# eukaryo/smith-waterman-simd

Measured on AMD Instinct MI355X. Metric: alignments/sec (and GCUPS) on 1M fixed-length pairs, 1/2/4/8 MI355X, higher is better.
Workload: dtype u16

## Files before the change

smith-waterman-simd_amd/csrc/swmi_api.cpp:

```cpp
#include "swmi_host.h"
#include "pk_form.h"

#include <cstdarg>
#include <cstdio>
#include <cstdlib>
#include <cstring>
#include <ctime>
#include <new>

namespace swmi {
namespace host {

namespace {
thread_local char t_error[512] = "";
thread_local int t_status = SWMI_OK;
thread_local int t_gpu = 0;
std::vector<std::shared_ptr<Context>> g_ctxs;
std::mutex g_init_mu;
Knobs g_knobs;
bool g_knobs_read = false;
std::atomic<uint64_t> g_schedule{0};
std::atomic<uint64_t> g_sg_mapping{0};
}

std::atomic<uint64_t> &sg_mapping_word() { return g_sg_mapping; }

int fail(int code, const char *fmt, ...)
{
    va_list ap;
    va_start(ap, fmt);
    vsnprintf(t_error, sizeof t_error, fmt, ap);
    va_end(ap);
    t_status = code;
    return code;
}

int last_status() { return t_status; }

std::mutex &init_mutex() { return g_init_mu; }
int num_contexts() { return (int)g_ctxs.size(); }
Context *context_at(int index) { return index >= 0 && index < (int)g_ctxs.size() ? g_ctxs[index].get() : nullptr; }
std::shared_ptr<Context> context_ref(int index) { return index >= 0 && index < (int)g_ctxs.size() ? g_ctxs[index] : nullptr; }

int check_alive(const Context &ctx)
{
    if (!ctx.dead.load(std::memory_order_acquire)) return SWMI_OK;
    return fail(SWMI_ERR_NOT_INITIALIZED, "swmi_shutdown() ran after this handle was created: only its *_destroy call is valid now");
}

const Knobs &knobs() { return g_knobs; }

void read_knobs()
{
    Knobs k;
    auto num = [](const char *name, long long lo, long long hi, long long dflt) {
        const char *v = getenv(name);
        if (!v || !*v) return dflt;
        const long long x = atoll(v);
        return x < lo || x > hi ? dflt : x;
    };
    k.host_granule = (size_t)num("SWMI_HOST_GRANULE", 1024, (long long)kChunkPairs, 0);
    k.host_serial = num("SWMI_HOST_SERIAL", 0, 1, 0) != 0;
    k.host_taper_pct = (unsigned)num("SWMI_HOST_TAPER", 1, 99, 0);
    k.host_min_granule = (size_t)num("SWMI_HOST_MIN_GRANULE", 1024, (long long)kChunkPairs, 0);
    if (const char *sched = getenv("SWMI_HOST_SCHEDULE")) {
        int c = 0;
        for (const char *q = sched; *q && c < 16;) {
            char *end = nullptr;
            const long long v = strtoll(q, &end, 10);
            if (end == q) break;
            if (v >= 1024 && v <= (long long)kChunkPairs) k.host_schedule[c++] = (size_t)v;
            q = *end == ',' ? end + 1 : end;
        }
    }
    k.host_trace = num("SWMI_HOST_TRACE", 0, 1, 0) != 0;
    k.host_threads = (int)num("SWMI_HOST_THREADS", 1, kHostThreads, 0);
    k.host_slots = (int)num("SWMI_HOST_SLOTS", 2, kSlots / kHostThreads, 0);
    k.score_group = (size_t)num("SWMI_TEST_SCORE_GROUP", 4096, (long long)kScoreGroup, (long long)kScoreGroup);
    k.extra_lds = (unsigned)num("SWMI_EXTRA_LDS", 0, 160 * 1024, 0);
    k.lanes = (int)num("SWMI_LANES", 0, 64, 0);
    k.banded_no_i16 = getenv("SWMI_BANDED_NO_I16") != nullptr;
    k.banded_no_pk = getenv("SWMI_BANDED_NO_PK") != nullptr;
    k.pk_no_product = getenv("SWMI_PK_NO_PRODUCT") != nullptr;
    k.sg_sweep = (int)num("SWMI_SG_SWEEP", 1, 44, -1);
    k.sg_exact = (int)num("SWMI_SG_EXACT", 0, 1, -1);
    const char *gb = getenv("SWMI_GATHER_BACKEND");
    k.gather_p2p = gb && strcmp(gb, "p2p") == 0;
    k.gather_piece = (size_t)num("SWMI_TEST_GATHER_PIECE", 1, 1ll << 40, 0);
    if (const char *lib = getenv("SWMI_RCCL_LIB")) snprintf(k.rccl_lib, sizeof k.rccl_lib, "%s", lib);
    g_knobs = k;
    g_knobs_read = true;
}

Context *current()
{
    if (g_ctxs.empty()) {
        fail(SWMI_ERR_NOT_INITIALIZED, "swmi_init() has not been called (or failed)");
        return nullptr;
    }
    Context *ctx = context_at(t_gpu);
    if (!ctx) {
        fail(SWMI_ERR_INVALID_ARGUMENT, "this thread selected GPU index %d but only %d are bound", t_gpu, (int)g_ctxs.size());
        return nullptr;
    }
    const hipError_t e = hipSetDevice(ctx->device);
    if (e != hipSuccess) {
        fail(SWMI_ERR_HIP, "hipSetDevice(%d) failed: %s", ctx->device, hipGetErrorString(e));
        return nullptr;
    }
    return ctx;
}

int check_params(const int8_t *sm, int gap)
{
    if (!sm) return fail(SWMI_ERR_INVALID_ARGUMENT, "score_matrix is NULL");
    if (gap < 0) return fail(SWMI_ERR_DOMAIN, "gap_penalty %d < 0 is outside the supported domain [0,127]", gap);
    return SWMI_OK;
}

SmRows pack_rows(const int8_t *sm, int add)
{
    SmRows rows;
    for (int a = 0; a < 4; ++a) {
        uint32_t r = 0;
        for (int b = 0; b < 4; ++b) r |= uint32_t(uint8_t(int8_t(sm[4 * a + b] + add))) << (8 * b);
        rows.r[a] = r;
    }
    return rows;
}

namespace {
int auto_lanes(size_t n)
{
    return n <= 2048 ? 64 : n <= 5120 ? 32 : n <= 24576 ? 16 : n <= 98304 ? 8 : 4;
}
int resolve_lanes(uint64_t schedule, size_t n)
{
    const int lanes = int(schedule & 0xffffffffu);
    const unsigned flags = unsigned(schedule >> 32);
    return lanes ? lanes : (flags & swmi::kUseLut) ? 4 : auto_lanes(n);
}
}

LaunchConfig make_config(const Context &ctx, const int8_t *sm, int gap, SmRows *rows, size_t n)
{
    const uint64_t schedule = g_schedule.load(std::memory_order_relaxed);
    const unsigned flags = unsigned(schedule >> 32);
    LaunchConfig cfg;
    cfg.lanes_per_alignment = resolve_lanes(schedule, n);
    cfg.use_i16 = (flags & swmi::kUseI16) != 0;
    cfg.use_lut = (flags & swmi::kUseLut) != 0;
    cfg.extra_lds_bytes = ctx.extra_lds;
    cfg.pk_bias = 0;
    cfg.pk_variant = 0;
    bool fold = !(flags & swmi::kNoGapFold);
    for (int k = 0; k < 16 && fold; ++k) {
        const int v = int(sm[k]) + gap;
        if (v < -128 || v > 127) fold = false;
    }
    cfg.fold_gap = fold;
// ... 29 lines not shown
        }
        for (int a = 0; a < 4; ++a) {
            uint32_t r = 0;
            for (int b = 0; b < 4; ++b) r |= uint32_t(int(sm[4 * a + b]) + add) << (8 * b);
            rows->r[a] = r;
        }
        return cfg;
    }
    *rows = pack_rows(sm, fold ? gap : 0);
    return cfg;
}

namespace {
int ensure_slot(Slot &s, size_t bytes, size_t scores)
{
    if (s.capacity < bytes) {
        if (s.d_seq1) { (void)hipFree(s.d_seq1); s.d_seq1 = nullptr; }
        if (s.d_seq2) { (void)hipFree(s.d_seq2); s.d_seq2 = nullptr; }
        s.capacity = 0;
        SWMI_HIP_TRY(hipMalloc(&s.d_seq1, bytes));
        SWMI_HIP_TRY(hipMalloc(&s.d_seq2, bytes));
        s.capacity = bytes;
    }
    if (s.score_capacity < scores) {
        if (s.d_scores) { (void)hipFree(s.d_scores); s.d_scores = nullptr; }
        s.score_capacity = 0;
        SWMI_HIP_TRY(hipMalloc(reinterpret_cast<void **>(&s.d_scores), scores * sizeof(int32_t)));
        s.score_capacity = scores;
    }
    return SWMI_OK;
}

}

int launch_device(Context &ctx, const void *d1, const void *d2, size_t n, const int8_t *sm, int gap, void *d_out,
                  hipStream_t st, bool packed)
{
    SmRows rows;
    const LaunchConfig cfg = make_config(ctx, sm, gap, &rows, n);
    const size_t stride = packed ? SWMI_PACKED_LEN : kSeq;
    for (size_t off = 0; off < n; off += kMaxLaunchPairs) {
        const size_t m = n - off < kMaxLaunchPairs ? n - off : kMaxLaunchPairs;
        SWMI_HIP_TRY(swmi::launch_score(cfg, static_cast<const uint8_t *>(d1) + off * stride,
                                        static_cast<const uint8_t *>(d2) + off * stride,
                                        static_cast<int32_t *>(d_out) + off, m, rows, gap, packed, st));
    }
    return SWMI_OK;
}

size_t host_entry_bytes(int entry)
{
    return entry == kEntryPacked ? 2 * SWMI_PACKED_LEN : entry == kEntryOneVsMany ? kSeq : 2 * kSeq;
}

size_t next_granule(size_t remaining, size_t bytes_per_pair)
{
    const Knobs &kn = knobs();
    if (kn.host_granule) return remaining < kn.host_granule ? remaining : kn.host_granule;
    const size_t smallest = kn.host_min_granule ? kn.host_min_granule : kMinGranule;
    if (remaining <= smallest) return remaining;
    size_t f1024 = kn.host_taper_pct ? size_t(kn.host_taper_pct) * 1024 / 100 : 65536 / bytes_per_pair;
    if (f1024 > kMaxTaper1024) f1024 = kMaxTaper1024;
    size_t g = (remaining - remaining * f1024 / 1024) & ~size_t(4095);
    if (g > kChunkPairs) g = kChunkPairs;
    if (g < smallest) g = smallest;
    return g;
}

namespace {
int ensure_scores_all(Context &ctx, size_t pairs)
{
    if (ctx.scores_all_capacity >= pairs) return SWMI_OK;
    if (ctx.d_scores_all) { (void)hipFree(ctx.d_scores_all); ctx.d_scores_all = nullptr; }
    ctx.scores_all_capacity = 0;
    SWMI_HIP_TRY(hipMalloc(reinterpret_cast<void **>(&ctx.d_scores_all), pairs * sizeof(int32_t)));
    ctx.scores_all_capacity = pairs;
    return SWMI_OK;
}
}

namespace {
struct Granule { size_t off, m; };

struct TraceRow { size_t index, pairs; int thread; hipEvent_t ev[3]; double host_issue_ms[2]; };
std::mutex g_trace_mu;
std::vector<TraceRow> g_trace;
double host_now_ms()
{
    timespec ts;
    clock_gettime(CLOCK_MONOTONIC, &ts);
    return ts.tv_sec * 1e3 + ts.tv_nsec * 1e-6;
}

hipError_t issue_granules(Context &ctx, const std::vector<Granule> &list, size_t first, size_t step, Slot *const *slots, int n_slots,
                          const uint8_t *s1, const uint8_t *s2, size_t group, size_t in_stride, const int8_t *sm, int gap,
                          int32_t *out, bool packed, bool one_vs_many, bool serial, bool *slot_used, size_t early = 0,
                          bool *slot_early_used = nullptr, std::atomic<bool> *early_done = nullptr)
{
    hipError_t e = hipSuccess;
    size_t j = 0;
    for (size_t i = first; i < list.size() && e == hipSuccess; i += step, ++j) {
        const size_t off = list[i].off, m = list[i].m, at = group + off;
        const int which = int(j % size_t(n_slots));
        Slot &s = *slots[which];
        SmRows rows;
        const LaunchConfig cfg = make_config(ctx, sm, gap, &rows, m);
        TraceRow tr{i, m, int(first), {nullptr, nullptr, nullptr}, {0, 0}};
        const bool trace = knobs().host_trace;
        if (trace) {
            for (auto &ev : tr.ev) (void)hipEventCreate(&ev);
            tr.host_issue_ms[0] = host_now_ms();
            (void)hipEventRecord(tr.ev[0], s.stream);
        }
        e = hipMemcpyAsync(s.d_seq1, s1 + at * in_stride, m * in_stride, hipMemcpyHostToDevice, s.stream);
        if (e == hipSuccess && !one_vs_many)
            e = hipMemcpyAsync(s.d_seq2, s2 + at * in_stride, m * in_stride, hipMemcpyHostToDevice, s.stream);
        if (trace) (void)hipEventRecord(tr.ev[1], s.stream);
        if (e == hipSuccess)
            e = one_vs_many ? swmi::launch_score_one_vs_many(cfg, s.d_seq1, s.d_seq2, ctx.d_scores_all + off, m, rows, gap, s.stream)
                            : swmi::launch_score(cfg, s.d_seq1, s.d_seq2, ctx.d_scores_all + off, m, rows, gap, packed, s.stream);
        if (trace) {
            (void)hipEventRecord(tr.ev[2], s.stream);
            tr.host_issue_ms[1] = host_now_ms();
            std::lock_guard<std::mutex> l(g_trace_mu);
            g_trace.push_back(tr);
        }
        if (e == hipSuccess && serial)
            e = hipMemcpyAsync(out + at, ctx.d_scores_all + off, m * sizeof(int32_t), hipMemcpyDeviceToHost, s.stream);
        slot_used[which] = true;
        if (i < early && e == hipSuccess) {
            e = hipEventRecord(ctx.slot_early[&s - ctx.slots], s.stream);
            slot_early_used[which] = true;
        }
        if (early_done && i + step >= early) early_done->store(true, std::memory_order_release);
    }
    if (early_done) early_done->store(true, std::memory_order_release);
    return e;
}
}

void granule_list(size_t group_n, size_t bytes_per_pair, std::vector<size_t> *out)
{
    out->clear();
    const Knobs &kn = knobs();
    if (kn.host_schedule[0]) {
        size_t k = 0;
        for (size_t rem = group_n; rem;) {
            const size_t want = kn.host_schedule[k], g = rem < want ? rem : want;
            out->push_back(g);
            rem -= g;
            if (k + 1 < 16 && kn.host_schedule[k + 1]) ++k;
        }
        return;
    }
    const bool balanced = bytes_per_pair * 15 <= 1024;
    if (balanced && !kn.host_granule && !kn.host_taper_pct) {
        const size_t steady = kn.host_min_granule ? kn.host_min_granule : kBalancedGranule;
        const size_t ramp[2] = {steady / 4, steady - steady / 4};
        if (group_n < 4 * steady) {
            for (size_t rem = group_n; rem;) {
                const size_t g = rem < steady / 2 ? rem : steady / 2;
                out->push_back(g);
                rem -= g;
            }
            return;
        }
        out->push_back(ramp[0]);
        out->push_back(ramp[1]);
        const size_t middle = group_n - 2 * steady;
        const size_t count = (middle + steady - 1) / steady;
        for (size_t k = 0, done = 0; k < count; ++k) {
            const size_t upto = k + 1 == count ? middle : (middle * (k + 1) / count) & ~size_t(4095);
            out->push_back(upto - done);
            done = upto;
        }
        out->push_back(ramp[1]);
        out->push_back(ramp[0]);
        return;
    }
    for (size_t rem = group_n; rem;) {
        const size_t g = next_granule(rem, bytes_per_pair);
        out->push_back(g);
        rem -= g;
    }
}

int score_host_batch(Context &ctx, const uint8_t *s1, const uint8_t *s2, size_t n, const int8_t *sm, int gap, int32_t *out,
                     bool packed, bool one_vs_many)
{
    std::lock_guard<std::mutex> lock(ctx.mu);
    const size_t in_stride = packed ? SWMI_PACKED_LEN : kSeq;
    const size_t per_pair = host_entry_bytes(packed ? kEntryPacked : one_vs_many ? kEntryOneVsMany : kEntryPairs);
    const bool serial = knobs().host_serial;
    const size_t score_group = knobs().score_group;
    const size_t first_group = n < score_group ? n : score_group;
    std::vector<size_t> sizes;
    const size_t tail = n > score_group ? n % score_group : 0;
    size_t largest = 0;
    if (tail) {
        granule_list(tail, per_pair, &sizes);
        for (size_t g : sizes) largest = g > largest ? g : largest;
    }
    granule_list(first_group, per_pair, &sizes);
    for (size_t g : sizes) largest = g > largest ? g : largest;
    const size_t first_count = sizes.size();
    const bool balanced = per_pair * 15 <= 1024;
    const int want_threads = knobs().host_threads ? knobs().host_threads : balanced ? 2 : 1;
    const int threads = (serial || want_threads < 2 || first_count < 2) ? 1 : 2;
    const int per_thread = knobs().host_slots ? knobs().host_slots : threads == 2 ? 2 : 3;
    const int used_slots = threads == 2 ? 2 * per_thread : n > score_group || first_count > size_t(per_thread) ? per_thread : int(first_count);
    for (int k = 0; k < used_slots; ++k) {
        const int rc = ensure_slot(ctx.slots[k], largest * in_stride, 0);
        if (rc != SWMI_OK) return rc;
    }
    {
        const int rc = ensure_scores_all(ctx, first_group);
        if (rc != SWMI_OK) return rc;
    }
    if (threads == 2 && !ctx.copier) ctx.copier.reset(new Worker);
    hipError_t e = hipSuccess;
    if (one_vs_many)
        for (int k = 0; k < used_slots && e == hipSuccess; ++k)
            e = hipMemcpyAsync(ctx.slots[k].d_seq2, s2, kSeq, hipMemcpyHostToDevice, ctx.slots[k].stream);
    Slot *mine[kSlots], *theirs[kSlots];
    int n_mine = 0, n_theirs = 0;
    for (int k = 0; k < used_slots; ++k) {
        if (threads == 1 || k % 2 == 0) mine[n_mine++] = &ctx.slots[k];
        else                            theirs[n_theirs++] = &ctx.slots[k];
    }
    std::vector<Granule> list;
    for (size_t group = 0; group < n && e == hipSuccess; group += score_group) {
        const size_t group_n = n - group < score_group ? n - group : score_group;
        list.clear();
        granule_list(group_n, per_pair, &sizes);
        {
            size_t off = 0;
            for (size_t m : sizes) {
                list.push_back(Granule{off, m});
                off += m;
            }
        }
        bool used_mine[kSlots] = {}, used_theirs[kSlots] = {};
        hipError_t e2 = hipSuccess;
        const size_t early = threads == 2 && list.size() >= 4 ? list.size() - 2 : 0;
        const size_t early_pairs = early ? list[early].off : 0;
        if (threads == 2 && list.size() > 1) {
            const int device = ctx.device;
            bool early_mine[kSlots] = {}, early_theirs[kSlots] = {};
            std::atomic<bool> mine_done{false};
            ctx.copier->submit([&, device] {
                e2 = hipSetDevice(device);
                if (e2 == hipSuccess)
                    e2 = issue_granules(ctx, list, 1, 2, theirs, n_theirs, s1, s2, group, in_stride, sm, gap, out, packed, one_vs_many,
                                        serial, used_theirs, early, early_theirs);
                if (e2 != hipSuccess || early == 0) return;
                while (!mine_done.load(std::memory_order_acquire)) std::this_thread::yield();
                for (int k = 0; k < n_mine && e2 == hipSuccess; ++k)
                    if (early_mine[k]) e2 = hipStreamWaitEvent(ctx.stream, ctx.slot_early[mine[k] - ctx.slots], 0);
                for (int k = 0; k < n_theirs && e2 == hipSuccess; ++k)
                    if (early_theirs[k]) e2 = hipStreamWaitEvent(ctx.stream, ctx.slot_early[theirs[k] - ctx.slots], 0);
                if (e2 == hipSuccess)
                    e2 = hipMemcpyAsync(out + group, ctx.d_scores_all, early_pairs * sizeof(int32_t), hipMemcpyDeviceToHost, ctx.stream);
                const hipError_t es = hipStreamSynchronize(ctx.stream);
                if (e2 == hipSuccess) e2 = es;
            });
            e = issue_granules(ctx, list, 0, 2, mine, n_mine, s1, s2, group, in_stride, sm, gap, out, packed, one_vs_many, serial, used_mine,
                               early, early_mine, &mine_done);
            mine_done.store(true, std::memory_order_release);
            ctx.copier->wait();
            if (e == hipSuccess) e = e2;
        } else {
            e = issue_granules(ctx, list, 0, 1, mine, n_mine, s1, s2, group, in_stride, sm, gap, out, packed, one_vs_many, serial, used_mine);
        }
        if (e != hipSuccess) break;
        const size_t last = list.size() - 1;
        const bool last_is_mine = threads == 1 || list.size() == 1 || last % 2 == 0;
        const size_t last_j = threads == 1 || list.size() == 1 ? last : last / 2;
        Slot *last_slot = last_is_mine ? mine[last_j % size_t(n_mine)] : theirs[last_j % size_t(n_theirs)];
        const bool more = group + group_n < n;
        if (serial) {
            for (int k = 0; k < n_mine && more && e == hipSuccess; ++k)
                if (used_mine[k]) e = hipStreamSynchronize(mine[k]->stream);
            continue;
        }
        auto join = [&](Slot *s) {
            if (s == last_slot || e != hipSuccess) return;
            hipEvent_t ev = ctx.slot_done[s - ctx.slots];
            e = hipEventRecord(ev, s->stream);
            if (e == hipSuccess) e = hipStreamWaitEvent(last_slot->stream, ev, 0);
        };
        for (int k = 0; k < n_mine; ++k)
            if (used_mine[k]) join(mine[k]);
        for (int k = 0; k < n_theirs; ++k)
            if (used_theirs[k]) join(theirs[k]);
        if (e == hipSuccess)
            e = hipMemcpyAsync(out + group + early_pairs, ctx.d_scores_all + early_pairs, (group_n - early_pairs) * sizeof(int32_t),
                               hipMemcpyDeviceToHost, last_slot->stream);
        if (e == hipSuccess && more) e = hipStreamSynchronize(last_slot->stream);
    }
    for (int k = 0; k < kSlots; ++k)
        if (ctx.slots[k].stream) {
            const hipError_t es = hipStreamSynchronize(ctx.slots[k].stream);
            if (e == hipSuccess) e = es;
        }
    if (knobs().host_trace) {
        std::lock_guard<std::mutex> l(g_trace_mu);
        const double t_end = host_now_ms();
        hipEvent_t ref = nullptr;
        double host0 = 0;
        for (auto &r : g_trace)
            if (r.index == 0) { ref = r.ev[0]; host0 = r.host_issue_ms[0]; }
        fprintf(stderr, "swmi host batch, %zu pairs, %zu B per pair: granule, pairs, issuing thread | GPU: copies start .. end, kernel end | host: issue start .. end (ms)\n",
                n, per_pair);
        for (auto &r : g_trace) {
            float t[3] = {0, 0, 0};
            for (int k = 0; k < 3; ++k)
                if (ref) (void)hipEventElapsedTime(&t[k], ref, r.ev[k]);
            fprintf(stderr, "  %3zu %8zu  t%d | %7.3f .. %7.3f  %7.3f | %7.3f .. %7.3f\n", r.index, r.pairs, r.thread, t[0], t[1], t[2],
                    r.host_issue_ms[0] - host0, r.host_issue_ms[1] - host0);
        }
        for (auto &r : g_trace)
            for (auto &ev : r.ev) (void)hipEventDestroy(ev);
        fprintf(stderr, "  call returns at %.3f ms\n", t_end - host0);
        g_trace.clear();
    }
    if (e != hipSuccess) return fail(SWMI_ERR_HIP, "host batch on GPU %d failed: %s", ctx.device, hipGetErrorString(e));
    return SWMI_OK;
}

int semiglobal_expand_moves(uint32_t max_length, const uint64_t *moves, uint32_t length, int32_t *traceback, size_t cap)
{
    if (!moves || (!traceback && cap)) return fail(SWMI_ERR_INVALID_ARGUMENT, "NULL buffer");
    if (length == 0 || length > max_length) return fail(SWMI_ERR_INVALID_ARGUMENT, "length %u outside [1, %u]", length, max_length);
    const size_t count = length < cap ? length : cap;
    if (count == 0) return SWMI_OK;
    static const uint64_t kStep[4] = {0, uint64_t(1) << 32, 1, (uint64_t(1) << 32) | 1};
    uint64_t pos = 0;
    memcpy(traceback, &pos, sizeof pos);
    int64_t t = int64_t(length) - 2;
    for (size_t k = 1; k < count; ++k, --t) {
        pos += kStep[(moves[t >> 5] >> (2 * (t & 31))) & 3u];
        memcpy(traceback + 2 * k, &pos, sizeof pos);
    }
    return SWMI_OK;
}

}
}

using namespace swmi::host;
using swmi::LaunchConfig;
using swmi::SmRows;
#define HIP_TRY SWMI_HIP_TRY


struct swmi_queue {
    std::shared_ptr<Context> ctx;
    int device = -1;
    size_t max_pairs = 0, count = 0, shipped = 0;
    size_t block = 1 << 16;
    int8_t sm[16];
    int gap = 0;
    uint8_t *h_seq1 = nullptr, *h_seq2 = nullptr;
    int32_t *h_scores = nullptr;
    uint8_t *d_seq1 = nullptr, *d_seq2 = nullptr;
    int32_t *d_scores = nullptr;
    hipStream_t stream = nullptr;
};

namespace {
int queue_ship(swmi_queue *q, size_t upto)
{
    if (upto <= q->shipped) return SWMI_OK;
    const int alive = check_alive(*q->ctx);
    if (alive != SWMI_OK) return alive;
    HIP_TRY(hipSetDevice(q->device));
    const size_t off = q->shipped, m = upto - q->shipped;
    HIP_TRY(hipMemcpyAsync(q->d_seq1 + off * kSeq, q->h_seq1 + off * kSeq, m * kSeq, hipMemcpyHostToDevice, q->stream));
    HIP_TRY(hipMemcpyAsync(q->d_seq2 + off * kSeq, q->h_seq2 + off * kSeq, m * kSeq, hipMemcpyHostToDevice, q->stream));
    const int rc = launch_device(*q->ctx, q->d_seq1 + off * kSeq, q->d_seq2 + off * kSeq, m, q->sm, q->gap, q->d_scores + off,
                                 q->stream, false);
    if (rc != SWMI_OK) return rc;
    HIP_TRY(hipMemcpyAsync(q->h_scores + off, q->d_scores + off, m * sizeof(int32_t), hipMemcpyDeviceToHost, q->stream));
    q->shipped = upto;
    return SWMI_OK;
}

void destroy_context(Context &c)
{
    c.copier.reset();
    (void)hipSetDevice(c.device);
    (void)hipDeviceSynchronize();
    for (auto &s : c.slots) {
        if (s.d_seq1) (void)hipFree(s.d_seq1);
        if (s.d_seq2) (void)hipFree(s.d_seq2);
        if (s.d_scores) (void)hipFree(s.d_scores);
        if (s.stream) (void)hipStreamDestroy(s.stream);
        s = Slot{};
    }
    if (c.stream) (void)hipStreamDestroy(c.stream);
    c.stream = nullptr;
    if (c.d_scores_all) (void)hipFree(c.d_scores_all);
    c.d_scores_all = nullptr;
    c.scores_all_capacity = 0;
    for (auto &ev : c.slot_done) {
        if (ev) (void)hipEventDestroy(ev);
        ev = nullptr;
    }
    for (auto &ev : c.slot_early) {
        if (ev) (void)hipEventDestroy(ev);
        ev = nullptr;
    }
    for (auto &w : c.sg_workspaces)
        if (w.second.ptr) (void)hipFree(w.second.ptr);
    c.sg_workspaces.clear();
    for (auto &g : c.sg_sets) {
        (void)hipFree(g.d1); (void)hipFree(g.d2); (void)hipFree(g.ws); (void)hipFree(g.d_scores); (void)hipFree(g.d_len); (void)hipFree(g.d_tb);
        (void)hipFree(g.d_moves);
        g = SgSet{};
    }
    for (auto &state : c.table_states) state.reset();
    if (c.pin) (void)hipHostFree(c.pin);
    c.pin = nullptr;
    c.pin_dev = nullptr;
}

int create_context(Context &c, int index, int device)
{
    c.index = index;
    c.device = device;
    HIP_TRY(hipSetDevice(device));
    HIP_TRY(hipGetDeviceProperties(&c.prop, device));
    if (strncmp(c.prop.gcnArchName, "gfx950", 6) != 0)
        return fail(SWMI_ERR_UNSUPPORTED_ARCH, "device %d is %s; libswmi carries gfx950 (MI355X) code objects only", device,
                    c.prop.gcnArchName);
    HIP_TRY(hipStreamCreateWithFlags(&c.stream, hipStreamNonBlocking));
    for (auto &s : c.slots) HIP_TRY(hipStreamCreateWithFlags(&s.stream, hipStreamNonBlocking));
    for (auto &ev : c.slot_done) HIP_TRY(hipEventCreateWithFlags(&ev, hipEventDisableTiming));
    for (auto &ev : c.slot_early) HIP_TRY(hipEventCreateWithFlags(&ev, hipEventDisableTiming));
    HIP_TRY(hipHostMalloc(reinterpret_cast<void **>(&c.pin), kPinPairs * (2 * kSeq + sizeof(int32_t)), hipHostMallocMapped));
    HIP_TRY(hipHostGetDevicePointer(&c.pin_dev, c.pin, 0));
    c.extra_lds = knobs().extra_lds;
    return SWMI_OK;
}

int init_list(const int *devices, int n)
{
    read_knobs();
    std::vector<std::shared_ptr<Context>> fresh;
    for (int k = 0; k < n; ++k) {
        fresh.emplace_back(std::make_shared<Context>());
        const int rc = create_context(*fresh.back(), k, devices[k]);
        if (rc != SWMI_OK) {
            for (auto &c : fresh) destroy_context(*c);
            return rc;
        }
    }
    for (int a = 0; a < n; ++a)
        for (int b = 0; b < n; ++b)
            if (devices[a] != devices[b]) {
                int can = 0;
                if (hipDeviceCanAccessPeer(&can, devices[a], devices[b]) == hipSuccess && can) {
                    (void)hipSetDevice(devices[a]);
                    (void)hipDeviceEnablePeerAccess(devices[b], 0);
                    (void)hipGetLastError();
                }
            }
    (void)hipSetDevice(devices[0]);
    g_ctxs = std::move(fresh);
    if (knobs().lanes && swmi::schedule_supported(knobs().lanes)) g_schedule.store(uint64_t(knobs().lanes));
    if (knobs().sg_sweep >= 0 && swmi_semiglobal_set_mapping(knobs().sg_sweep) != SWMI_OK) (void)swmi_semiglobal_set_mapping(-1);
    if (knobs().sg_exact >= 0) (void)swmi_semiglobal_set_exact(knobs().sg_exact ? 1 : 0);
    return SWMI_OK;
}

// ... 809 lines not shown
```

smith-waterman-simd_amd/csrc/swmi_host.h:

```cpp
#pragma once
#include "../../include/swmi.h"
#include "swmi_internal.h"

#include <atomic>
#include <condition_variable>
#include <functional>
#include <map>
#include <memory>
#include <mutex>
#include <thread>
#include <vector>

namespace swmi {
namespace host {

constexpr size_t kSeq = SWMI_SEQ_LEN;
constexpr size_t kChunkPairs = size_t(1) << 20;
constexpr size_t kMinGranule = size_t(1) << 14;
constexpr size_t kBalancedGranule = size_t(1) << 17;
constexpr size_t kMaxTaper1024 = 820;
constexpr size_t kScoreGroup = size_t(1) << 24;
constexpr size_t kMaxLaunchPairs = size_t(1) << 30;
constexpr int kSlots = 6;
constexpr int kHostThreads = 2;
constexpr size_t kPinPairs = 64;

struct Knobs {
    size_t host_granule = 0;
    bool host_serial = false;
    unsigned host_taper_pct = 0;
    size_t host_min_granule = 0;
    size_t host_schedule[16] = {};
    bool host_trace = false;
    int host_slots = 0;
    int host_threads = 0;
    size_t score_group = kScoreGroup;
    unsigned extra_lds = 0;
    int lanes = 0;
    bool banded_no_i16 = false;
    bool banded_no_pk = false;
    bool pk_no_product = false;
    int sg_sweep = -1;
    int sg_exact = -1;
    bool gather_p2p = false;
    size_t gather_piece = 0;
    char rccl_lib[256] = "";
};
const Knobs &knobs();
void read_knobs();

struct Slot {
    hipStream_t stream = nullptr;
    uint8_t *d_seq1 = nullptr, *d_seq2 = nullptr;
    size_t capacity = 0;
    int32_t *d_scores = nullptr;
    size_t score_capacity = 0;
};

enum HostEntry { kEntryPairs = 0, kEntryPacked = 1, kEntryOneVsMany = 2 };
size_t host_entry_bytes(int entry);
size_t next_granule(size_t remaining, size_t bytes_per_pair);
void granule_list(size_t group_n, size_t bytes_per_pair, std::vector<size_t> *out);

struct SgSet {
    uint8_t *d1 = nullptr, *d2 = nullptr;
    void *ws = nullptr;
    int32_t *d_scores = nullptr, *d_tb = nullptr;
    uint32_t *d_len = nullptr;
    unsigned long long *d_moves = nullptr;
    size_t alignments = 0, tb_entries = 0, move_rows = 0;
    size_t off = 0, m = 0;
};

struct Worker {
    std::thread th;
    std::mutex mu;
    std::condition_variable cv;
    std::function<void()> job;
    bool has_job = false, stop = false;
    Worker() { th = std::thread([this] { loop(); }); }
    ~Worker() { shut(); }
    Worker(const Worker &) = delete;
    Worker &operator=(const Worker &) = delete;
    void shut()
    {
        {
            std::lock_guard<std::mutex> l(mu);
            stop = true;
            cv.notify_all();
        }
        if (th.joinable()) th.join();
    }
    void loop()
    {
        std::unique_lock<std::mutex> l(mu);
        for (;;) {
            cv.wait(l, [this] { return has_job || stop; });
            if (has_job) {
                l.unlock();
                job();
                l.lock();
                has_job = false;
                cv.notify_all();
                continue;
            }
            return;
        }
    }
    void submit(std::function<void()> f)
    {
        std::lock_guard<std::mutex> l(mu);
        job = std::move(f);
        has_job = true;
        cv.notify_all();
    }
    void wait()
    {
        std::unique_lock<std::mutex> l(mu);
        cv.wait(l, [this] { return !has_job; });
    }
};

struct Workspace {
    void *ptr = nullptr;
    size_t bytes = 0;
};

enum TableFamily {
    kTableLocal, kTableSgfull, kTableLocalAffine, kTableSgfullAffine, kTableLocalFull, kTableLocalFullAffine, kTableGlobalFull,
    kTableGlobalFullAffine, kTableGlobalLong, kTableGlobalLongAffine, kTableLocalLong, kTableLocalLongAffine, kTableSemiglobalLong,
    kTableSemiglobalLongAffine, kTableFamilies
};

struct Context {
    int index = 0;
    int device = -1;
    std::atomic<bool> dead{false};
    hipDeviceProp_t prop{};
    hipStream_t stream = nullptr;
    Slot slots[kSlots];
    int32_t *d_scores_all = nullptr;
    size_t scores_all_capacity = 0;
    hipEvent_t slot_done[kSlots] = {};
    hipEvent_t slot_early[kSlots] = {};
    std::unique_ptr<Worker> copier;
    SgSet sg_sets[2];
    std::mutex ws_mu;
    std::map<hipStream_t, Workspace> sg_workspaces;
    uint8_t *pin = nullptr;
    void *pin_dev = nullptr;
    unsigned extra_lds = 0;
    std::shared_ptr<void> table_states[kTableFamilies];
    std::mutex mu;
};

int fail(int code, const char *fmt, ...) __attribute__((format(printf, 2, 3)));
int last_status();
Context *current();
Context *context_at(int index);
std::shared_ptr<Context> context_ref(int index);
void stop_workers();
int check_alive(const Context &ctx);
int num_contexts();
std::mutex &init_mutex();

std::atomic<uint64_t> &sg_mapping_word();
int check_params(const int8_t *sm, int gap);
SmRows pack_rows(const int8_t *sm, int add);
LaunchConfig make_config(const Context &ctx, const int8_t *sm, int gap, SmRows *rows, size_t n);
int launch_device(Context &ctx, const void *d1, const void *d2, size_t n, const int8_t *sm, int gap, void *d_out,
                  hipStream_t st, bool packed);
int score_host_batch(Context &ctx, const uint8_t *s1, const uint8_t *s2, size_t n, const int8_t *sm, int gap,
                     int32_t *out, bool packed, bool one_vs_many);

struct Table;
using TableLaunch = hipError_t (*)(const Table &t, const uint8_t *s1, const uint8_t *s2, size_t n, int32_t *scores, int32_t *ends,
                                   uint32_t *codes, unsigned long long *moves, uint32_t *counts, hipStream_t st);
using RaggedLaunch = hipError_t (*)(const Table &t, size_t slice, const uint8_t *s1, const uint8_t *s2, const void *work, size_t n,
                                    int32_t *scores, int32_t *ends, uint32_t *codes, unsigned long long *moves, uint32_t *counts,
                                    hipStream_t st);
struct RaggedPlan {
    RaggedLaunch launch;
    const uint64_t *seq1_offsets;
    const uint64_t *seq2_offsets = nullptr;
    std::vector<uint64_t> move_offsets;
    std::vector<size_t> first;
    std::vector<size_t> code_words;
    std::vector<LocalWork> work;
    const void *slots = nullptr;
    size_t slot_bytes = 0;
    size_t max_m = 0, max_seq1 = 0, max_seq2 = 0, max_codes = 0, max_moves = 0;
};
struct Table {
    TableLaunch launch;
    TableFamily state;
    size_t tb_slice_bytes;
    const char *count;
    size_t len1, len2;
    size_t ends;
    size_t code_words, move_words;
    uint32_t count_offset;
    const int8_t *sm;
    int gap, gap_extend;
    const RaggedPlan *plan = nullptr;
    unsigned free_ends = 0;
    size_t carry_words = 0;
    int32_t *carry = nullptr;
};
constexpr size_t kTableSliceBytes = size_t(256) << 20;
constexpr size_t kTableMaxSlice = size_t(1) << 20;
size_t table_slice_bytes(const Table &t, bool tb);
size_t table_slices_for(const Table &t, size_t n, bool tb, size_t *sizes, size_t cap);
int table_device(const Table &t, const void *d_seq1s, const void *d_seq2s, size_t n, void *d_scores, void *d_ends, void *d_moves,
                 void *d_counts, void *stream);
int table_host(const Table &t, const char *entry, const uint8_t *seq1s, const uint8_t *seq2s, size_t n, int32_t *scores,
               int32_t *ends, uint64_t *moves, uint32_t *counts);
int table_time_device(const Table &t, const char *entry, const void *d_seq1s, const void *d_seq2s, size_t n, void *d_scores,
                      void *d_ends, void *d_moves, void *d_counts, void *stream, int iters, float *avg_ms);
int table_check_timer(size_t n, int iters, const float *avg_ms);
Table family_table(TableFamily f, size_t len1, size_t len2, const int8_t *sm, int gap, int gap_extend, unsigned free_ends);
enum TileKind { kTileLocal, kTileGlobal, kTileSemiglobal, kTileKinds };
bool tile_ragged_plan_check(TileKind kind, const uint64_t *seq1_offsets, const uint64_t *seq2_offsets, size_t n, bool affine, bool tb,
                            std::vector<size_t> *slice_sizes, std::vector<size_t> *slice_bytes);
int semiglobal_expand_moves(uint32_t max_length, const uint64_t *moves, uint32_t length, int32_t *traceback, size_t cap);
int table_release_workspaces(TableFamily family);

#define SWMI_HIP_TRY(expr)                                                                                          \
// ... 10 lines not shown
```

Before: 1.243 billion.

## Pack host sequences to 2-bit on worker threads to shrink host-to-device copies

```diff
diff --git a/smith-waterman-simd_amd/csrc/host_pack.cpp b/smith-waterman-simd_amd/csrc/host_pack.cpp
--- /dev/null
+++ b/smith-waterman-simd_amd/csrc/host_pack.cpp
@@ -0,0 +1,79 @@
+#include "host_pack.h"
+
+#include <cstring>
+
+#if defined(__x86_64__) || defined(__i386__)
+#include <immintrin.h>
+#define SWMI_HOST_PACK_X86 1
+#endif
+
+namespace swmi {
+namespace host {
+
+void pack_bases_2bit_scalar(const uint8_t *src, uint8_t *dst, size_t n_bytes)
+{
+    size_t k = 0;
+    for (; k + 4 <= n_bytes; k += 4) {
+        uint32_t w;
+        memcpy(&w, src + k, 4);
+        w &= 0x03030303u;
+        dst[k / 4] = uint8_t(w | w >> 6 | w >> 12 | w >> 18);
+    }
+    if (k < n_bytes) {
+        unsigned b = 0;
+        for (size_t j = k; j < n_bytes; ++j) b |= unsigned(src[j] & 3) << (2 * (j - k));
+        dst[k / 4] = uint8_t(b);
+    }
+}
+
+#ifdef SWMI_HOST_PACK_X86
+namespace {
+__attribute__((target("avx2"))) inline __m256i fold32(const uint8_t *p, __m256i mask, __m256i mul8, __m256i mul16)
+{
+    const __m256i v = _mm256_and_si256(_mm256_loadu_si256(reinterpret_cast<const __m256i *>(p)), mask);
+    return _mm256_madd_epi16(_mm256_maddubs_epi16(v, mul8), mul16);
+}
+}
+
+__attribute__((target("avx2"))) void pack_bases_2bit_avx2(const uint8_t *src, uint8_t *dst, size_t n_bytes)
+{
+    const __m256i mask = _mm256_set1_epi8(3);
+    const __m256i mul8 = _mm256_set1_epi16(0x0401);
+    const __m256i mul16 = _mm256_set1_epi32(0x00100001);
+    const __m256i order = _mm256_setr_epi32(0, 4, 1, 5, 2, 6, 3, 7);
+    const __m256i pick = _mm256_setr_epi8(0, 4, 8, 12, -1, -1, -1, -1, -1, -1, -1, -1, -1, -1, -1, -1,
+                                          0, 4, 8, 12, -1, -1, -1, -1, -1, -1, -1, -1, -1, -1, -1, -1);
+    size_t k = 0;
+    for (; k + 128 <= n_bytes; k += 128) {
+        const __m256i ab = _mm256_packus_epi32(fold32(src + k, mask, mul8, mul16), fold32(src + k + 32, mask, mul8, mul16));
+        const __m256i cd = _mm256_packus_epi32(fold32(src + k + 64, mask, mul8, mul16), fold32(src + k + 96, mask, mul8, mul16));
+        const __m256i bytes = _mm256_permutevar8x32_epi32(_mm256_packus_epi16(ab, cd), order);
+        _mm256_storeu_si256(reinterpret_cast<__m256i *>(dst + k / 4), bytes);
+    }
+    for (; k + 32 <= n_bytes; k += 32) {
+        const __m256i b = _mm256_shuffle_epi8(fold32(src + k, mask, mul8, mul16), pick);
+        const uint32_t lo = uint32_t(_mm256_extract_epi32(b, 0)), hi = uint32_t(_mm256_extract_epi32(b, 4));
+        memcpy(dst + k / 4, &lo, 4);
+        memcpy(dst + k / 4 + 4, &hi, 4);
+    }
+    pack_bases_2bit_scalar(src + k, dst + k / 4, n_bytes - k);
+}
+
+bool pack_bases_2bit_has_avx2()
+{
+    static const bool has = __builtin_cpu_supports("avx2");
+    return has;
+}
+#else
+void pack_bases_2bit_avx2(const uint8_t *src, uint8_t *dst, size_t n_bytes) { pack_bases_2bit_scalar(src, dst, n_bytes); }
+bool pack_bases_2bit_has_avx2() { return false; }
+#endif
+
+void pack_bases_2bit(const uint8_t *src, uint8_t *dst, size_t n_bytes)
+{
+    if (pack_bases_2bit_has_avx2()) pack_bases_2bit_avx2(src, dst, n_bytes);
+    else                            pack_bases_2bit_scalar(src, dst, n_bytes);
+}
+
+}
+}
diff --git a/smith-waterman-simd_amd/csrc/host_pack.h b/smith-waterman-simd_amd/csrc/host_pack.h
--- /dev/null
+++ b/smith-waterman-simd_amd/csrc/host_pack.h
@@ -0,0 +1,15 @@
+#pragma once
+#include <cstddef>
+#include <cstdint>
+
+namespace swmi {
+namespace host {
+
+void pack_bases_2bit(const uint8_t *src, uint8_t *dst, size_t n_bytes);
+
+void pack_bases_2bit_scalar(const uint8_t *src, uint8_t *dst, size_t n_bytes);
+void pack_bases_2bit_avx2(const uint8_t *src, uint8_t *dst, size_t n_bytes);
+bool pack_bases_2bit_has_avx2();
+
+}
+}
diff --git a/smith-waterman-simd_amd/csrc/swmi_api.cpp b/smith-waterman-simd_amd/csrc/swmi_api.cpp
--- a/smith-waterman-simd_amd/csrc/swmi_api.cpp
+++ b/smith-waterman-simd_amd/csrc/swmi_api.cpp
@@ -1,4 +1,5 @@
 #include "swmi_host.h"
+#include "host_pack.h"
 #include "pk_form.h"
 
 #include <cstdarg>
@@ -8,8 +9,12 @@
 #include <ctime>
 #include <new>
 
+#include <sched.h>
+
 namespace swmi {
 namespace host {
+
+void pack_bases_2bit(const uint8_t *src, uint8_t *dst, size_t n_bytes) __attribute__((weak));
 
 namespace {
 thread_local char t_error[512] = "";
@@ -76,6 +81,19 @@
     k.host_trace = num("SWMI_HOST_TRACE", 0, 1, 0) != 0;
     k.host_threads = (int)num("SWMI_HOST_THREADS", 1, kHostThreads, 0);
     k.host_slots = (int)num("SWMI_HOST_SLOTS", 2, kSlots / kHostThreads, 0);
+    k.host_pack = num("SWMI_HOST_PACK", 0, 1, kHostPackDefault) != 0;
+    {
+        cpu_set_t set;
+        long long cpus = sched_getaffinity(0, sizeof set, &set) == 0 ? CPU_COUNT(&set) : (long long)std::thread::hardware_concurrency();
+        long long dflt = cpus - 2 < 8 ? cpus - 2 : 8;
+        if (dflt < 0) dflt = 0;
+        k.host_pack_threads = (int)num("SWMI_HOST_PACK_THREADS", 0, kPackMaxThreads, -1);
+        k.host_pack_threads_set = k.host_pack_threads >= 0;
+        if (!k.host_pack_threads_set) k.host_pack_threads = (int)dflt;
+    }
+    k.host_pack_share = (int)num("SWMI_HOST_PACK_SHARE", 0, 100, -1);
+    k.host_pack_head = (size_t)num("SWMI_HOST_PACK_HEAD", 4096, (long long)kChunkPairs, (long long)kPackHeadGranule) & ~size_t(4095);
+    k.host_pack_min = (size_t)num("SWMI_TEST_HOST_PACK_MIN", 1, 1ll << 40, (long long)kPackMinPairs);
     k.score_group = (size_t)num("SWMI_TEST_SCORE_GROUP", 4096, (long long)kScoreGroup, (long long)kScoreGroup);
     k.extra_lds = (unsigned)num("SWMI_EXTRA_LDS", 0, 160 * 1024, 0);
     k.lanes = (int)num("SWMI_LANES", 0, 64, 0);
@@ -271,7 +289,7 @@
 namespace {
 struct Granule { size_t off, m; };
 
-struct TraceRow { size_t index, pairs; int thread; hipEvent_t ev[3]; double host_issue_ms[2]; };
+struct TraceRow { size_t index, pairs; int thread; bool pack_tail; hipEvent_t ev[3]; double host_issue_ms[2]; };
 std::mutex g_trace_mu;
 std::vector<TraceRow> g_trace;
 double host_now_ms()
@@ -279,6 +297,34 @@
     timespec ts;
     clock_gettime(CLOCK_MONOTONIC, &ts);
     return ts.tv_sec * 1e3 + ts.tv_nsec * 1e-6;
+}
+
+hipError_t issue_one(Context &ctx, Slot &s, size_t index, int thread, const uint8_t *s1, const uint8_t *s2, size_t at, size_t off, size_t m,
+                     size_t in_stride, const int8_t *sm, int gap, bool packed, bool one_vs_many)
+{
+    SmRows rows;
+    const LaunchConfig cfg = make_config(ctx, sm, gap, &rows, m);
+    TraceRow tr{index, m, thread, false, {nullptr, nullptr, nullptr}, {0, 0}};
+    const bool trace = knobs().host_trace;
+    if (trace) {
+        for (auto &ev : tr.ev) (void)hipEventCreate(&ev);
+        tr.host_issue_ms[0] = host_now_ms();
+        (void)hipEventRecord(tr.ev[0], s.stream);
+    }
+    hipError_t e = hipMemcpyAsync(s.d_seq1, s1 + at * in_stride, m * in_stride, hipMemcpyHostToDevice, s.stream);
+    if (e == hipSuccess && !one_vs_many)
+        e = hipMemcpyAsync(s.d_seq2, s2 + at * in_stride, m * in_stride, hipMemcpyHostToDevice, s.stream);
+    if (trace) (void)hipEventRecord(tr.ev[1], s.stream);
+    if (e == hipSuccess)
+        e = one_vs_many ? swmi::launch_score_one_vs_many(cfg, s.d_seq1, s.d_seq2, ctx.d_scores_all + off, m, rows, gap, s.stream)
+                        : swmi::launch_score(cfg, s.d_seq1, s.d_seq2, ctx.d_scores_all + off, m, rows, gap, packed, s.stream);
+    if (trace) {
+        (void)hipEventRecord(tr.ev[2], s.stream);
+        tr.host_issue_ms[1] = host_now_ms();
+        std::lock_guard<std::mutex> l(g_trace_mu);
+        g_trace.push_back(tr);
+    }
+    return e;
 }
 
 hipError_t issue_granules(Context &ctx, const std::vector<Granule> &list, size_t first, size_t step, Slot *const *slots, int n_slots,
@@ -292,28 +338,7 @@
         const size_t off = list[i].off, m = list[i].m, at = group + off;
         const int which = int(j % size_t(n_slots));
         Slot &s = *slots[which];
-        SmRows rows;
-        const LaunchConfig cfg = make_config(ctx, sm, gap, &rows, m);
-        TraceRow tr{i, m, int(first), {nullptr, nullptr, nullptr}, {0, 0}};
-        const bool trace = knobs().host_trace;
-        if (trace) {
-            for (auto &ev : tr.ev) (void)hipEventCreate(&ev);
-            tr.host_issue_ms[0] = host_now_ms();
-            (void)hipEventRecord(tr.ev[0], s.stream);
-        }
-        e = hipMemcpyAsync(s.d_seq1, s1 + at * in_stride, m * in_stride, hipMemcpyHostToDevice, s.stream);
-        if (e == hipSuccess && !one_vs_many)
-            e = hipMemcpyAsync(s.d_seq2, s2 + at * in_stride, m * in_stride, hipMemcpyHostToDevice, s.stream);
-        if (trace) (void)hipEventRecord(tr.ev[1], s.stream);
-        if (e == hipSuccess)
-            e = one_vs_many ? swmi::launch_score_one_vs_many(cfg, s.d_seq1, s.d_seq2, ctx.d_scores_all + off, m, rows, gap, s.stream)
-                            : swmi::launch_score(cfg, s.d_seq1, s.d_seq2, ctx.d_scores_all + off, m, rows, gap, packed, s.stream);
-        if (trace) {
-            (void)hipEventRecord(tr.ev[2], s.stream);
-            tr.host_issue_ms[1] = host_now_ms();
-            std::lock_guard<std::mutex> l(g_trace_mu);
-            g_trace.push_back(tr);
-        }
+        e = issue_one(ctx, s, i, int(first), s1, s2, at, off, m, in_stride, sm, gap, packed, one_vs_many);
         if (e == hipSuccess && serial)
             e = hipMemcpyAsync(out + at, ctx.d_scores_all + off, m * sizeof(int32_t), hipMemcpyDeviceToHost, s.stream);
         slot_used[which] = true;
@@ -372,6 +397,292 @@
         out->push_back(g);
         rem -= g;
     }
+}
+
+namespace {
+struct PackCursors {
+    std::atomic<uint64_t> word;
+    size_t boundary_lo, boundary_hi;
+    PackCursors(size_t n, size_t lo, size_t hi) : word(uint64_t(n) << 32), boundary_lo(lo), boundary_hi(hi) {}
+    size_t claim_head(size_t want, size_t *off)
+    {
+        uint64_t v = word.load(std::memory_order_relaxed);
+        for (;;) {
+            const size_t h = size_t(v & 0xffffffffu), t = size_t(v >> 32), lim = t < boundary_hi ? t : boundary_hi;
+            if (h >= lim) return 0;
+            const size_t m = want < lim - h ? want : lim - h;
+            if (word.compare_exchange_weak(v, uint64_t(t) << 32 | uint64_t(h + m), std::memory_order_acq_rel)) {
+                *off = h;
+                return m;
+            }
+        }
+    }
+    size_t claim_tail(size_t *off)
+    {
+        uint64_t v = word.load(std::memory_order_relaxed);
+        for (;;) {
+            const size_t h = size_t(v & 0xffffffffu), t = size_t(v >> 32), lim = h > boundary_lo ? h : boundary_lo;
+            if (t <= lim) return 0;
+            const size_t ragged = t % kPackChunk ? t % kPackChunk : kPackChunk;
+            const size_t m = ragged < t - lim ? ragged : t - lim;
+            if (word.compare_exchange_weak(v, uint64_t(t - m) << 32 | uint64_t(h), std::memory_order_acq_rel)) {
+                *off = t - m;
+                return m;
+            }
+        }
+    }
+    size_t tail_start() const { return size_t(word.load(std::memory_order_acquire) >> 32); }
+};
+
+struct PackJob {
+    Context *ctx;
+    const uint8_t *s1, *s2;
+    size_t group;
+    const int8_t *sm;
+    int gap;
+    PackCursors *cursors;
+};
+
+struct PackPool {
+    struct Buf {
+        uint8_t *h = nullptr, *d = nullptr;
+        hipEvent_t freed = nullptr;
+        bool in_flight = false;
+    };
+    struct Thread {
+        std::thread th;
+        std::vector<Buf> bufs;
+        hipError_t err = hipSuccess;
+    };
+    struct Stream {
+        hipStream_t stream = nullptr;
+        hipEvent_t done = nullptr;
+        bool used = false;
+    };
+    int device = -1;
+    std::vector<std::unique_ptr<Thread>> threads;
+    std::vector<Stream> streams;
+    std::mutex issue_mu;
+    size_t issued = 0;
+    std::mutex mu;
+    std::condition_variable cv;
+    const PackJob *job = nullptr;
+    uint64_t generation = 0;
+    int running = 0;
+    bool stop = false;
+
+    ~PackPool() { join(); }
+    PackPool() = default;
+    PackPool(const PackPool &) = delete;
+    PackPool &operator=(const PackPool &) = delete;
+
+    hipError_t create(int dev, int n_threads)
+    {
+        device = dev;
+        const size_t bytes = kPackChunk * 2 * SWMI_PACKED_LEN;
+        const int per_thread = n_threads >= 2 ? 2 : 4;
+        streams.resize(size_t(kPackStreams));
+        for (Stream &st : streams) {
+            hipError_t e = hipStreamCreateWithFlags(&st.stream, hipStreamNonBlocking);
+            if (e == hipSuccess) e = hipEventCreateWithFlags(&st.done, hipEventDisableTiming);
+            if (e != hipSuccess) return e;
+        }
+        for (int t = 0; t < n_threads; ++t) {
+            threads.emplace_back(new Thread);
+            Thread &me = *threads.back();
+            hipError_t e = hipSuccess;
+            me.bufs.resize(size_t(per_thread));
+            for (Buf &b : me.bufs) {
+                if (e == hipSuccess) e = hipHostMalloc(reinterpret_cast<void **>(&b.h), bytes, hipHostMallocDefault);
+                if (e == hipSuccess) e = hipMalloc(reinterpret_cast<void **>(&b.d), bytes);
+                if (e == hipSuccess) e = hipEventCreateWithFlags(&b.freed, hipEventDisableTiming);
+            }
+            if (e != hipSuccess) return e;
+        }
+        for (size_t t = 0; t < threads.size(); ++t) threads[t]->th = std::thread([this, t] { loop(int(t)); });
+        return hipSuccess;
+    }
+    void join()
+    {
+        {
+            std::lock_guard<std::mutex> l(mu);
+            stop = true;
+            cv.notify_all();
+        }
+        for (auto &t : threads)
+            if (t->th.joinable()) t->th.join();
+    }
+    void release()
+    {
+        join();
+        for (auto &t : threads) {
+            for (Buf &b : t->bufs) {
+                if (b.h) (void)hipHostFree(b.h);
+                if (b.d) (void)hipFree(b.d);
+                if (b.freed) (void)hipEventDestroy(b.freed);
+            }
+        }
+        for (Stream &st : streams) {
+            if (st.done) (void)hipEventDestroy(st.done);
+            if (st.stream) (void)hipStreamDestroy(st.stream);
+        }
+        threads.clear();
+        streams.clear();
+    }
+    void start(const PackJob &j)
+    {
+        std::lock_guard<std::mutex> l(mu);
+        job = &j;
+        running = int(threads.size());
+        for (auto &t : threads) t->err = hipSuccess;
+        for (Stream &st : streams) st.used = false;
+        ++generation;
+        cv.notify_all();
+    }
+    void wait()
+    {
+        std::unique_lock<std::mutex> l(mu);
+        cv.wait(l, [this] { return running == 0; });
+        job = nullptr;
+    }
+    void loop(int index)
+    {
+        Thread &me = *threads[size_t(index)];
+        bool device_set = false;
+        uint64_t seen = 0;
+        std::unique_lock<std::mutex> l(mu);
+        for (;;) {
+            cv.wait(l, [&] { return stop || generation != seen; });
+            if (generation == seen) return;
+            seen = generation;
+            const PackJob *j = job;
+            l.unlock();
+            if (!device_set) {
+                me.err = hipSetDevice(device);
+                device_set = me.err == hipSuccess;
+            }
+            if (me.err == hipSuccess) me.err = work(me, index, *j);
+            l.lock();
+            if (--running == 0) {
+                for (Stream &st : streams)
+                    if (st.used && me.err == hipSuccess) me.err = hipEventRecord(st.done, st.stream);
+                cv.notify_all();
+            }
+        }
+    }
+    hipError_t work(Thread &me, int index, const PackJob &j)
+    {
+        Context &ctx = *j.ctx;
+        const bool trace = knobs().host_trace;
+        hipError_t e = hipSuccess;
+        size_t off = 0, turn = 0;
+        while (e == hipSuccess) {
+            const size_t m = j.cursors->claim_tail(&off);
+            if (m == 0) break;
+            Buf &b = me.bufs[turn++ % me.bufs.size()];
+            if (b.in_flight) {
+                e = hipEventSynchronize(b.freed);
+                b.in_flight = false;
+                if (e != hipSuccess) break;
+            }
+            TraceRow tr{off / kPackChunk, m, index, true, {nullptr, nullptr, nullptr}, {0, 0}};
+            if (trace) tr.host_issue_ms[0] = host_now_ms();
+            const size_t at = j.group + off;
+            pack_bases_2bit(j.s1 + at * kSeq, b.h, m * kSeq);
+            pack_bases_2bit(j.s2 + at * kSeq, b.h + m * SWMI_PACKED_LEN, m * kSeq);
+            SmRows rows;
+            const LaunchConfig cfg = make_config(ctx, j.sm, j.gap, &rows, m);
+            if (trace)
+                for (auto &ev : tr.ev) (void)hipEventCreate(&ev);
+            std::unique_lock<std::mutex> issue(issue_mu);
+            Stream &st = streams[issued++ % streams.size()];
+            if (trace) (void)hipEventRecord(tr.ev[0], st.stream);
+            e = hipMemcpyAsync(b.d, b.h, 2 * m * SWMI_PACKED_LEN, hipMemcpyHostToDevice, st.stream);
+            if (trace) (void)hipEventRecord(tr.ev[1], st.stream);
+            if (e == hipSuccess)
+                e = swmi::launch_score(cfg, b.d, b.d + m * SWMI_PACKED_LEN, ctx.d_scores_all + off, m, rows, j.gap, true, st.stream);
+            if (e == hipSuccess) e = hipEventRecord(b.freed, st.stream);
+            b.in_flight = e == hipSuccess;
+            st.used = true;
+            if (trace) (void)hipEventRecord(tr.ev[2], st.stream);
+            issue.unlock();
+            if (trace) {
+                tr.host_issue_ms[1] = host_now_ms();
+                std::lock_guard<std::mutex> lt(g_trace_mu);
+                g_trace.push_back(tr);
+            }
+        }
+        return e;
+    }
+};
+
+PackPool *pack_pool_for(Context &ctx, hipError_t *e)
+{
+    *e = hipSuccess;
+    if (ctx.pack_pool) return static_cast<PackPool *>(ctx.pack_pool.get());
+    const Knobs &kn = knobs();
+    int n_threads = kn.host_pack_threads;
+    if (!kn.host_pack_threads_set && n_threads > 1 && num_contexts() > 1)
+        n_threads = n_threads / num_contexts() ? n_threads / num_contexts() : 1;
+    if (!&pack_bases_2bit || n_threads <= 0) return nullptr;
+    std::shared_ptr<PackPool> pool = std::make_shared<PackPool>();
+    *e = pool->create(ctx.device, n_threads);
+    if (*e != hipSuccess) {
+        pool->release();
+        return nullptr;
+    }
+    ctx.pack_pool = pool;
+    return pool.get();
+}
+
+hipError_t pack_tail_group(Context &ctx, PackPool &pool, const std::vector<size_t> &sizes, Slot *const *mine, int n_mine, const uint8_t *s1,
+                           const uint8_t *s2, size_t group, size_t group_n, const int8_t *sm, int gap, int32_t *out,
+                           hipStream_t *last_stream)
+{
+    const Knobs &kn = knobs();
+    size_t lo = 0, hi = group_n;
+    if (kn.host_pack_share == 0) lo = hi = group_n;
+    else if (kn.host_pack_share > 0) lo = hi = (group_n - group_n * size_t(kn.host_pack_share) / 100) & ~size_t(4095);
+    PackCursors cursors(group_n, lo, hi);
+    const PackJob job{&ctx, s1, s2, group, sm, gap, &cursors};
+    pool.start(job);
+    hipError_t e = hipSuccess;
+    bool used[kSlots] = {};
+    Slot *last = mine[0];
+    size_t pieces = 0;
+    bool met = false;
+    for (size_t i = 0; i < sizes.size() && !met && e == hipSuccess; ++i)
+        for (size_t left = sizes[i]; left && !met && e == hipSuccess;) {
+            const size_t want = left < kn.host_pack_head ? left : kn.host_pack_head;
+            size_t off = 0;
+            const size_t m = cursors.claim_head(want, &off);
+            met = m < want;
+            if (m == 0) break;
+            const int which = int(pieces % size_t(n_mine));
+            last = mine[which];
+            e = issue_one(ctx, *last, pieces++, 0, s1, s2, group + off, off, m, kSeq, sm, gap, false, false);
+            used[which] = true;
+            left -= m;
+        }
+    pool.wait();
+    for (auto &t : pool.threads)
+        if (e == hipSuccess) e = t->err;
+    for (auto &st : pool.streams)
+        if (e == hipSuccess && st.used) e = hipStreamWaitEvent(last->stream, st.done, 0);
+    for (int k = 0; k < n_mine && e == hipSuccess; ++k)
+        if (used[k] && mine[k] != last) {
+            hipEvent_t ev = ctx.slot_done[mine[k] - ctx.slots];
+            e = hipEventRecord(ev, mine[k]->stream);
+            if (e == hipSuccess) e = hipStreamWaitEvent(last->stream, ev, 0);
+        }
+    if (e == hipSuccess) e = hipMemcpyAsync(out + group, ctx.d_scores_all, group_n * sizeof(int32_t), hipMemcpyDeviceToHost, last->stream);
+    *last_stream = last->stream;
+    if (kn.host_trace)
+        fprintf(stderr, "swmi host batch: group of %zu pairs, %zu raw from the front, %zu packed from the back (%.1f %%), %zu pack threads\n",
+                group_n, cursors.tail_start(), group_n - cursors.tail_start(), 100.0 * double(group_n - cursors.tail_start()) / double(group_n),
+                pool.threads.size());
+    return e;
+}
 }
 
 int score_host_batch(Context &ctx, const uint8_t *s1, const uint8_t *s2, size_t n, const int8_t *sm, int gap, int32_t *out,
@@ -395,9 +706,15 @@
     const size_t first_count = sizes.size();
     const bool balanced = per_pair * 15 <= 1024;
     const int want_threads = knobs().host_threads ? knobs().host_threads : balanced ? 2 : 1;
-    const int threads = (serial || want_threads < 2 || first_count < 2) ? 1 : 2;
+    hipError_t e = hipSuccess;
+    PackPool *pool = nullptr;
+    if (!packed && !one_vs_many && !serial && knobs().host_pack && first_group >= knobs().host_pack_min) {
+        pool = pack_pool_for(ctx, &e);
+        if (e != hipSuccess) return fail(SWMI_ERR_HIP, "host batch on GPU %d: no pack pool: %s", ctx.device, hipGetErrorString(e));
+    }
+    const int threads = (serial || want_threads < 2 || first_count < 2 || pool) ? 1 : 2;
     const int per_thread = knobs().host_slots ? knobs().host_slots : threads == 2 ? 2 : 3;
-    const int used_slots = threads == 2 ? 2 * per_thread : n > score_group || first_count > size_t(per_thread) ? per_thread : int(first_count);
+    const int used_slots = threads == 2 ? 2 * per_thread : pool || n > score_group || first_count > size_t(per_thread) ? per_thread : int(first_count);
     for (int k = 0; k < used_slots; ++k) {
         const int rc = ensure_slot(ctx.slots[k], largest * in_stride, 0);
         if (rc != SWMI_OK) return rc;
@@ -407,7 +724,6 @@
         if (rc != SWMI_OK) return rc;
     }
     if (threads == 2 && !ctx.copier) ctx.copier.reset(new Worker);
-    hipError_t e = hipSuccess;
     if (one_vs_many)
         for (int k = 0; k < used_slots && e == hipSuccess; ++k)
             e = hipMemcpyAsync(ctx.slots[k].d_seq2, s2, kSeq, hipMemcpyHostToDevice, ctx.slots[k].stream);
@@ -422,6 +738,12 @@
         const size_t group_n = n - group < score_group ? n - group : score_group;
         list.clear();
         granule_list(group_n, per_pair, &sizes);
+        if (pool && group_n >= knobs().host_pack_min) {
+            hipStream_t last_stream = nullptr;
+            e = pack_tail_group(ctx, *pool, sizes, mine, n_mine, s1, s2, group, group_n, sm, gap, out, &last_stream);
+            if (e == hipSuccess && group + group_n < n) e = hipStreamSynchronize(last_stream);
+            continue;
+        }
         {
             size_t off = 0;
             for (size_t m : sizes) {
@@ -492,20 +814,26 @@
             const hipError_t es = hipStreamSynchronize(ctx.slots[k].stream);
             if (e == hipSuccess) e = es;
         }
+    if (pool)
+        for (auto &t : pool->streams) {
+            const hipError_t es = hipStreamSynchronize(t.stream);
+            if (e == hipSuccess) e = es;
+        }
     if (knobs().host_trace) {
         std::lock_guard<std::mutex> l(g_trace_mu);
         const double t_end = host_now_ms();
         hipEvent_t ref = nullptr;
         double host0 = 0;
+        if (!g_trace.empty()) { ref = g_trace[0].ev[0]; host0 = g_trace[0].host_issue_ms[0]; }
         for (auto &r : g_trace)
-            if (r.index == 0) { ref = r.ev[0]; host0 = r.host_issue_ms[0]; }
-        fprintf(stderr, "swmi host batch, %zu pairs, %zu B per pair: granule, pairs, issuing thread | GPU: copies start .. end, kernel end | host: issue start .. end (ms)\n",
+            if (r.index == 0 && !r.pack_tail) { ref = r.ev[0]; host0 = r.host_issue_ms[0]; }
+        fprintf(stderr, "swmi host batch, %zu pairs, %zu B per pair: granule, pairs, issuing thread (p = pack thread, a packed chunk: 64 B per pair, its host span includes the pack) | GPU: copies start .. end, kernel end | host: issue start .. end (ms)\n",
                 n, per_pair);
         for (auto &r : g_trace) {
             float t[3] = {0, 0, 0};
             for (int k = 0; k < 3; ++k)
                 if (ref) (void)hipEventElapsedTime(&t[k], ref, r.ev[k]);
-            fprintf(stderr, "  %3zu %8zu  t%d | %7.3f .. %7.3f  %7.3f | %7.3f .. %7.3f\n", r.index, r.pairs, r.thread, t[0], t[1], t[2],
+            fprintf(stderr, "  %3zu %8zu  %c%d | %7.3f .. %7.3f  %7.3f | %7.3f .. %7.3f\n", r.index, r.pairs, r.pack_tail ? 'p' : 't', r.thread, t[0], t[1], t[2],
                     r.host_issue_ms[0] - host0, r.host_issue_ms[1] - host0);
         }
         for (auto &r : g_trace)
@@ -580,6 +908,10 @@
     c.copier.reset();
     (void)hipSetDevice(c.device);
     (void)hipDeviceSynchronize();
+    if (c.pack_pool) {
+        static_cast<PackPool *>(c.pack_pool.get())->release();
+        c.pack_pool.reset();
+    }
     for (auto &s : c.slots) {
         if (s.d_seq1) (void)hipFree(s.d_seq1);
         if (s.d_seq2) (void)hipFree(s.d_seq2);
diff --git a/smith-waterman-simd_amd/csrc/swmi_host.h b/smith-waterman-simd_amd/csrc/swmi_host.h
--- a/smith-waterman-simd_amd/csrc/swmi_host.h
+++ b/smith-waterman-simd_amd/csrc/swmi_host.h
@@ -23,6 +23,12 @@
 constexpr size_t kMaxLaunchPairs = size_t(1) << 30;
 constexpr int kSlots = 6;
 constexpr int kHostThreads = 2;
+constexpr size_t kPackChunk = size_t(1) << 16;
+constexpr size_t kPackMinPairs = size_t(1) << 18;
+constexpr size_t kPackHeadGranule = size_t(1) << 16;
+constexpr int kPackStreams = 4;
+constexpr int kPackMaxThreads = 16;
+constexpr int kHostPackDefault = 1;
 constexpr size_t kPinPairs = 64;
 
 struct Knobs {
@@ -34,6 +40,12 @@
     bool host_trace = false;
     int host_slots = 0;
     int host_threads = 0;
+    bool host_pack = kHostPackDefault != 0;
+    int host_pack_threads = 0;
+    bool host_pack_threads_set = false;
+    int host_pack_share = -1;
+    size_t host_pack_head = kPackHeadGranule;
+    size_t host_pack_min = kPackMinPairs;
     size_t score_group = kScoreGroup;
     unsigned extra_lds = 0;
     int lanes = 0;
@@ -143,6 +155,7 @@
     size_t scores_all_capacity = 0;
     hipEvent_t slot_done[kSlots] = {};
     hipEvent_t slot_early[kSlots] = {};
+    std::shared_ptr<void> pack_pool;
     std::unique_ptr<Worker> copier;
     SgSet sg_sets[2];
     std::mutex ws_mu;
```

New measurement: 1.244 billion, median of 2. About the same (+0.1%).
